# flanglet/kanzi-cpp

Hardware: AMD Instinct MI355X
Metric: encode+decode MB/s on the synthetic stand-in for silesia.tar (bit-exact) (higher is better)
Workload: dtype u8

## Files before the change

kanzi-cpp_amd/csrc/bwt_fwd.hip:

```cpp
#include "common.hpp"
#include "stages.hpp"
#include "bwt_common.hpp"

#include <cstdlib>
#include <cstring>
#include <algorithm>
#include <cmath>
#include "prims.hpp"
#include <chrono>
#include <vector>

namespace knz {

constexpr u32 SM_TS = 1792;
constexpr u32 SM_WIN = 2048;
constexpr u32 SM_G = 256;
constexpr u32 MED_CAP = 8192;
constexpr u32 MED_LO_CAP = 2048;
constexpr u32 SUPER_CAP = 8192;
constexpr int GATHER_THREADS = 512;
constexpr u32 GATHER_ROWS = 16;
static_assert(MED_CAP <= GATHER_ROWS * GATHER_THREADS, "k_bwt_f_gather_desc judges a medium group from one batch of loads");
constexpr u32 LARGE_OS_MIN = 1000000;
constexpr u32 NO_BIT = 0x7FFFFFFFu;
// ... 904 lines not shown
        else for (u32 i0 = 0; i0 < d.y; i0 += GATHER_ROWS * GATHER_THREADS)
            unsplit = gather_rows<(int)GATHER_ROWS>(v, d.x + i0, d.y - i0, off, bb, be, judge, key0, &sDiff);
        if (threadIdx.x == 0) {
            descInfo[g] = make_uint2(bb, lab);
            if (unsplit) {
                v.medStage[d.x >> 8] = d; desc[g] = make_uint2(d.x, 0u);
                if (v.verdictNow) v.verdictNow[d.x >> 8] = make_uint2(key0, verdict_word(v.round, (off == h && key0 != 0u) ? VERDICT_PLAIN : VERDICT_WHOLE, d.y));
            }
            if (stats) {
                atomicAdd(&v.counters[CNT_STAT_MED], d.y); atomicAdd(&v.counters[CNT_STAT_MED_GROUPS], 1u);
                if (unsplit) { atomicAdd(&v.counters[CNT_STAT_UNSPLIT], 1u); atomicAdd(&v.counters[CNT_STAT_UNSPLIT_MEMBERS], d.y); }
            }
        }
        __syncthreads();
    }
}

__device__ __forceinline__ bool sleep_target(const FwdView& v, const uint2* __restrict__ desc, u32 nDesc, u32 lab, u32 bb, bool plain, u32& start, u32& key)
{
    u32 lo = 0, hi = nDesc;
    while (lo < hi) { const u32 mid = (lo + hi) >> 1; if (desc[mid].x <= lab) lo = mid + 1; else hi = mid; }
    if (lo == 0) return false;
    start = desc[lo - 1].x;
    const uint2 t = v.verdictWas[start >> 8];
    const u32 status = (t.y >> 16) & 3u;
    if ((t.y >> 24) != v.round - 1u || (plain ? status != VERDICT_PLAIN : status == 0u) || lab - start >= (t.y & 0xFFFFu)) return false;
    key = t.x;
    return lab_old(v, v.SA[start], bb) == lab;
}

__global__ __launch_bounds__(256) void k_bwt_f_med_sleep(FwdView v, uint2* __restrict__ desc, u32 nDesc, int stats)
{
    const u32 g = blockIdx.x * 256 + threadIdx.x;
    if (g >= nDesc) return;
    const uint2 d = desc[g];
    if (d.y <= SM_G || d.y > MED_CAP) return;
    const uint2 was = v.verdictWas[d.x >> 8];
    if (was.y != verdict_word(v.round - 1u, VERDICT_PLAIN, d.y)) return;
    if (v.rtbits && ((v.rtbits[d.x >> 5] >> (d.x & 31)) & 1u)) return;
    const u32 bb = v.base[find_block(v.base, v.nBlocks, d.x)];
    u32 s1, k1, s2, k2;
    if (!sleep_target(v, desc, nDesc, bb + was.x - 1u, bb, true, s1, k1) || s1 == d.x) return;
    if (!sleep_target(v, desc, nDesc, bb + k1 - 1u, bb, false, s2, k2) || s2 == d.x) return;
    v.verdictNow[d.x >> 8] = make_uint2(k1, verdict_word(v.round, VERDICT_PLAIN, d.y));
    v.medStage[d.x >> 8] = d;
    desc[g] = make_uint2(d.x, 0u);
    if (stats) {
        atomicAdd(&v.counters[CNT_STAT_MED], d.y); atomicAdd(&v.counters[CNT_STAT_MED_GROUPS], 1u);
        atomicAdd(&v.counters[CNT_STAT_UNSPLIT], 1u); atomicAdd(&v.counters[CNT_STAT_UNSPLIT_MEMBERS], d.y);
        atomicAdd(&v.counters[CNT_STAT_ASLEEP], 1u); atomicAdd(&v.counters[CNT_STAT_ASLEEP_MEMBERS], d.y);
    }
}

template <int THREADS, int ROWS>
struct MedLds {
    static constexpr int WAVES = THREADS / 64;
    static constexpr u32 CAP = (u32)ROWS * THREADS;
    u32 oK[CAP];
    u32 oV[CAP];
    u32 cnt[WAVES * 256];
    u32 fb[CAP / 32];
    int pm[CAP / 32];
    u32 pn[CAP / 32];
    u32 wtot[WAVES];
    u32 wtot2[WAVES];
    u32 oldLab;
    u32 blkBase;
};

template <int THREADS, int ROWS>
__device__ __forceinline__ u32 med_block_sum(MedLds<THREADS, ROWS>& L, u32 x)
{
    const u32 s = wave_sum(x);
    if ((threadIdx.x & 63) == 0) L.wtot[threadIdx.x >> 6] = s;
    __syncthreads();
    u32 tot = 0;
    for (int w = 0; w < THREADS / 64; w++) tot += L.wtot[w];
    __syncthreads();
    return tot;
}

template <int THREADS, int ROWS>
__device__ __forceinline__ void med_radix_sort(MedLds<THREADS, ROWS>& L, u32 n, int npass)
{
    constexpr int WAVES = THREADS / 64;
    const int tid = (int)threadIdx.x, lane = tid & 63, wave = tid >> 6;
    const unsigned long long ltMask = (lane == 0) ? 0ull : (~0ull >> (64 - lane));
    u32* cntw = L.cnt + wave * 256;
    const int R = (int)((n + THREADS - 1) / THREADS);
    const u32 waveBase = (u32)wave * (u32)R * 64u;
    for (int pass = 0; pass < npass; pass++) {
        const int shift = 8 * pass;
        for (int q = lane; q < 256; q += 64) cntw[q] = 0;
        u32 key[ROWS], val[ROWS], pre[ROWS];
#pragma unroll
        for (int r = 0; r < ROWS; r++) {
            key[r] = 0xFFFFFFFFu; val[r] = 0; pre[r] = 0;
            if (r < R) {
                const u32 idx = waveBase + (u32)r * 64u + (u32)lane;
                if (idx < n) { key[r] = L.oK[idx]; val[r] = L.oV[idx]; }
                const u32 dg = (key[r] >> shift) & 255u;
                const unsigned long long peers = prims::digit_peers_fast(true, dg);
                const u32 pop = (u32)__popcll(peers);
                const u32 rnk = (u32)__popcll(peers & ltMask);
                const int leader = __ffsll((long long)peers) - 1;
                u32 old = 0;
                if (lane == leader) { old = cntw[dg]; cntw[dg] = old + pop; }
                old = (u32)__shfl((int)old, leader, 64);
                pre[r] = old + rnk;
            }
        }
        __syncthreads();
        {
            constexpr int TPD = THREADS / 256;
            const int dg = tid / TPD, w0 = (tid % TPD) * 4;
            const u32 c0 = L.cnt[(w0 + 0) * 256 + dg], c1 = L.cnt[(w0 + 1) * 256 + dg], c2 = L.cnt[(w0 + 2) * 256 + dg], c3 = L.cnt[(w0 + 3) * 256 + dg];
            const u32 sum = c0 + c1 + c2 + c3;
            const u32 incl = wave_incl_scan(sum);
            if (lane == 63) L.wtot[wave] = incl;
            __syncthreads();
            u32 wbase = 0;
            for (int w = 0; w < wave; w++) wbase += L.wtot[w];
            const u32 excl = wbase + incl - sum;
            L.cnt[(w0 + 0) * 256 + dg] = excl;
            L.cnt[(w0 + 1) * 256 + dg] = excl + c0;
            L.cnt[(w0 + 2) * 256 + dg] = excl + c0 + c1;
            L.cnt[(w0 + 3) * 256 + dg] = excl + c0 + c1 + c2;
        }
        __syncthreads();
#pragma unroll
        for (int r = 0; r < ROWS; r++) {
            if (r < R) {
                const u32 dg = (key[r] >> shift) & 255u;
                const u32 pos = cntw[dg] + pre[r];
                if (pos < n) {
                    L.oK[pos] = key[r];
                    L.oV[pos] = val[r];
                }
            }
        }
        __syncthreads();
    }
    (void)WAVES;
}

template <int THREADS, int ROWS>
__device__ __forceinline__ void med_write_back(MedLds<THREADS, ROWS>& L, const FwdView& v, u32 gs, u32 n, uint2* __restrict__ medNext, uint2* __restrict__ largeNext)
{
    constexpr u32 CAP = (u32)ROWS * THREADS;
    const int tid = (int)threadIdx.x, lane = tid & 63;
    const int nWords = (int)((n + 31) >> 5);
    if (tid < (int)(CAP / 32)) {
        u32 bits = 0;
        if (tid < nWords) {
            const u32 i0 = (u32)tid * 32u;
            u32 prev = (i0 == 0) ? 0u : L.oK[i0 - 1];
            for (u32 k = 0; k < 32; k++) {
                const u32 i = i0 + k;
                if (i >= n) break;
                const u32 cur = L.oK[i];
                if (i == 0 || cur != prev) bits |= 1u << k;
                prev = cur;
            }
        }
        L.fb[tid] = bits;
        L.pm[tid] = bits ? (tid * 32 + 31 - __clz((int)bits)) : -1;
        L.pn[tid] = bits ? (u32)(tid * 32 + __ffs((int)bits) - 1) : n;
    }
    __syncthreads();
    if (tid < 64) {
        constexpr int WPL = (int)(CAP / 32) / 64;
        int run = -1;
        for (int k = 0; k < WPL; k++) { const int x = L.pm[tid * WPL + k]; run = x > run ? x : run; }
        int incl = run;
        for (int o = 1; o < 64; o <<= 1) { const int t = __shfl_up(incl, (unsigned)o, 64); if (tid >= o) incl = t > incl ? t : incl; }
        int carry = __shfl_up(incl, 1u, 64);
        if (tid == 0) carry = -1;
        for (int k = 0; k < WPL; k++) { const int x = L.pm[tid * WPL + k]; carry = x > carry ? x : carry; L.pm[tid * WPL + k] = carry; }
        u32 runn = n;
        for (int k = WPL - 1; k >= 0; k--) { const u32 x = L.pn[tid * WPL + k]; runn = x < runn ? x : runn; }
        u32 incn = runn;
        for (int o = 1; o < 64; o <<= 1) { const u32 t = (u32)__shfl_down((int)incn, (unsigned)o, 64); if (tid + o < 64) incn = t < incn ? t : incn; }
        u32 carn = (u32)__shfl_down((int)incn, 1u, 64);
        if (tid == 63) carn = n;
        for (int k = WPL - 1; k >= 0; k--) { const u32 x = L.pn[tid * WPL + k]; carn = x < carn ? x : carn; L.pn[tid * WPL + k] = carn; }
    }
    __syncthreads();
    u32 surv = 0;
    const u32 oldLab = L.oldLab;
    __shared__ ClassAgg A;
    agg_init(A);
    __syncthreads();
    int hKind[ROWS];
    u32 hLocal[ROWS], hSize[ROWS];
#pragma unroll
    for (int r = 0; r < ROWS; r++) hKind[r] = -1;
    int row = 0;
    for (u32 i = (u32)tid; i < n; i += THREADS, row++) {
        const u32 w = i >> 5, bit = i & 31;
        const u32 lowmask = (bit == 31) ? 0xFFFFFFFFu : ((2u << bit) - 1u);
        const u32 word = L.fb[w];
        const u32 mm = word & lowmask;
        const u32 hd = mm ? (w * 32 + 31 - (u32)__clz((int)mm)) : (u32)L.pm[w - 1];
// ... 19 lines not shown
        if (hKind[r] >= 0) agg_write(A, v, hKind[r], hLocal[r], gs + (u32)tid + (u32)r * THREADS, hSize[r], largeNext, (uint2*)nullptr);
    if (tid < nWords && L.fb[tid]) {
        const u32 off = gs + (u32)tid * 32u;
        const u32 sh = off & 31;
        atomicOr(&v.gnew[off >> 5], L.fb[tid] << sh);
        if (sh && (L.fb[tid] >> (32 - sh))) atomicOr(&v.gnew[(off >> 5) + 1], L.fb[tid] >> (32 - sh));
    }
}

template <int THREADS, int ROWS>
__device__ __forceinline__ void med_majority_write_back(MedLds<THREADS, ROWS>& L, const FwdView& v, u32 gs, u32 n, u32 nOth, u32 c, u32 less, u32 m)
{
    const int tid = (int)threadIdx.x;
    const u32 oldLab = L.oldLab;
    (void)n; (void)m;
    const u32 mStart = gs + less;
    const u32 rel = oldLab - gs;
    const u32 mLab = (c <= SM_G) ? mStart : ((rel >= less && rel < less + c) ? oldLab : mStart + (c >> 1));
    for (u32 i = (u32)tid; i < c; i += THREADS) {
        const u32 gp = L.oV[nOth + i];
        v.SA[mStart + i] = gp;
        if (mLab != oldLab) lab_set(v, gp, L.blkBase, mLab, oldLab);
    }
    u32 surv = 0;
    if (tid == 0) {
        if (less != 0) atomicOr(&v.gnew[mStart >> 5], 1u << (mStart & 31));
        if (c > SM_G) v.medStage[mStart >> 8] = make_uint2(mStart, c);
        else if (c > 1) surv = 1;
    }
    if ((u32)tid < nOth) {
        const u32 t = (u32)tid;
        const u32 key = L.oK[t];
        u32 hd = t, e = t + 1;
        while (hd > 0 && L.oK[hd - 1] == key) hd--;
        while (e < nOth && L.oK[e] == key) e++;
        const u32 size = e - hd;
        const u32 shift = (t < less) ? 0u : c;
        const u32 slot = gs + t + shift, hdSlot = gs + hd + shift;
        const u32 relO = rel - shift;
        const u32 lab = (size <= SM_G) ? hdSlot : ((oldLab >= hdSlot && oldLab < hdSlot + size) ? oldLab : hdSlot + (size >> 1));
        (void)relO;
        const u32 gp = L.oV[t];
        v.SA[slot] = gp;
        if (lab != oldLab) lab_set(v, gp, L.blkBase, lab, oldLab);
        if (t == hd) {
            if (hdSlot != gs) atomicOr(&v.gnew[hdSlot >> 5], 1u << (hdSlot & 31));
            if (size > SM_G) v.medStage[hdSlot >> 8] = make_uint2(hdSlot, size);
            else if (size > 1) surv = 1;
        }
    }
    if (__ballot(surv != 0) != 0 && (tid & 63) == 0) v.counters[CNT_SMALL_LEFT] = 1;
}

template <int THREADS, int ROWS, bool STATS>
__device__ __forceinline__ void med_sort_group(MedLds<THREADS, ROWS>& L, const FwdView& v, u32 gs, u32 n, uint2 info, int npass, bool storeKeys,
                                               uint2* __restrict__ medNext, uint2* __restrict__ largeNext, uint4* __restrict__ superList)
{
    constexpr int WAVES = THREADS / 64;
    const int tid = (int)threadIdx.x, lane = tid & 63, wave = tid >> 6;
    const unsigned long long ltMask = (lane == 0) ? 0ull : (~0ull >> (64 - lane));
    if (tid == 0) { L.oldLab = info.y; L.blkBase = info.x; }
    const u32 ka = L.oK[n >> 2], kb = L.oK[n >> 1], kc = L.oK[(n >> 2) * 3];
    const u32 m = (ka == kc) ? ka : kb;
    u32 c = 0;
    for (u32 i = (u32)tid; i < n; i += THREADS) c += (L.oK[i] == m) ? 1u : 0u;
    c = med_block_sum(L, c);
    if (c < n && 2 * c >= n && n <= SUPER_CAP && m == info.y - info.x + 1u) {
        if (tid == 0) { const u32 at = atomicAdd(&v.counters[CNT_SUPER], 1u); superList[at] = make_uint4(gs, n, info.x, info.y); }
        if (storeKeys) for (u32 i = (u32)tid; i < n; i += THREADS) v.K[gs + i] = L.oK[i];
        __syncthreads();
        return;
    }
    if (STATS && tid == 0 && c == n) { atomicAdd(&v.counters[CNT_STAT_UNSPLIT], 1u); atomicAdd(&v.counters[CNT_STAT_UNSPLIT_MEMBERS], n); }
    if (c < n) {
        if (2 * c >= n) {
            const int R = (int)((n + THREADS - 1) / THREADS);
            const u32 waveBase = (u32)wave * (u32)R * 64u;
            u32 key[ROWS], val[ROWS], pos[ROWS];
            u32 runO = 0, runE = 0;
#pragma unroll
            for (int r = 0; r < ROWS; r++) {
                key[r] = m; val[r] = 0; pos[r] = 0xFFFFFFFFu;
                if (r < R) {
                    const u32 idx = waveBase + (u32)r * 64u + (u32)lane;
                    const bool valid = idx < n;
                    if (valid) { key[r] = L.oK[idx]; val[r] = L.oV[idx]; }
                    const bool oth = valid && key[r] != m, same = valid && key[r] == m;
                    const unsigned long long bo = __ballot(oth), be = __ballot(same);
                    if (oth) pos[r] = runO + (u32)__popcll(bo & ltMask);
                    if (same) pos[r] = 0x80000000u | (runE + (u32)__popcll(be & ltMask));
                    runO += (u32)__popcll(bo);
                    runE += (u32)__popcll(be);
                }
            }
            if (lane == 0) { L.wtot[wave] = runO; L.wtot2[wave] = runE; }
            __syncthreads();
            u32 baseO = 0, baseE = 0, nOth = 0;
            for (int w = 0; w < WAVES; w++) { if (w < wave) { baseO += L.wtot[w]; baseE += L.wtot2[w]; } nOth += L.wtot[w]; }
#pragma unroll
            for (int r = 0; r < ROWS; r++) {
                if (r < R && pos[r] != 0xFFFFFFFFu) {
                    const u32 at = (pos[r] & 0x80000000u) ? (nOth + baseE + (pos[r] & 0x7FFFFFFFu)) : (baseO + pos[r]);
                    L.oK[at] = key[r];
                    L.oV[at] = val[r];
                }
            }
            __syncthreads();
            if (nOth <= (u32)THREADS) {
                u32 kk = 0, vv = 0, at = 0;
                if ((u32)tid < nOth) {
                    kk = L.oK[tid]; vv = L.oV[tid];
                    for (u32 j = 0; j < nOth; j++) { const u32 kj = L.oK[j]; at += (kj < kk || (kj == kk && j < (u32)tid)) ? 1u : 0u; }
                }
                __syncthreads();
                if ((u32)tid < nOth) { L.oK[at] = kk; L.oV[at] = vv; }
                __syncthreads();
                u32 lessQ = 0;
                if ((u32)tid < nOth) lessQ = (L.oK[tid] < m) ? 1u : 0u;
                lessQ = med_block_sum(L, lessQ);
                if (tid == 0) { L.oldLab = info.y; L.blkBase = info.x; if (STATS) { atomicAdd(&v.counters[CNT_STAT_MAJ], 1u); atomicAdd(&v.counters[CNT_STAT_MAJ_MEMBERS], n); } }
                __syncthreads();
                med_majority_write_back<THREADS, ROWS>(L, v, gs, n, nOth, c, lessQ, m);
                __syncthreads();
                return;
            } else {
                med_radix_sort<THREADS, ROWS>(L, nOth, npass);
            }
            u32 less = 0;
            for (u32 i = (u32)tid; i < nOth; i += THREADS) less += (L.oK[i] < m) ? 1u : 0u;
            less = med_block_sum(L, less);
#pragma unroll
            for (int k = 0; k < ROWS; k++) {
                const u32 i = (u32)tid + (u32)k * THREADS;
                if (i < n) { key[k] = L.oK[i]; val[k] = L.oV[i]; }
            }
            __syncthreads();
#pragma unroll
            for (int k = 0; k < ROWS; k++) {
                const u32 i = (u32)tid + (u32)k * THREADS;
                if (i < n) {
                    const u32 at = (i < less) ? i : (i < nOth ? i + c : less + (i - nOth));
                    L.oK[at] = key[k];
                    L.oV[at] = val[k];
                }
            }
            __syncthreads();
        } else {
            med_radix_sort<THREADS, ROWS>(L, n, npass);
        }
    }
    med_write_back<THREADS, ROWS>(L, v, gs, n, medNext, largeNext);
    __syncthreads();
}

template <int THREADS, int ROWS, bool STATS>
__global__ __launch_bounds__(THREADS, (THREADS >= 1024 ? 4 : THREADS / 128)) void k_bwt_f_sort_medium(FwdView v, const uint2* __restrict__ desc, u32 nDesc, int npass, u32 minLen,
                                                               uint2* __restrict__ medNext, uint2* __restrict__ largeNext, const uint2* __restrict__ descInfo,
                                                               uint4* __restrict__ superList)
{
    constexpr u32 CAP = (u32)ROWS * THREADS;
    __shared__ MedLds<THREADS, ROWS> L;
    const int tid = (int)threadIdx.x;

    for (u32 g = blockIdx.x; g < nDesc; g += gridDim.x) {
        const uint2 d = desc[g];
        const u32 gs = d.x, n = d.y;
        if (n <= minLen || n > CAP) continue;
        const uint2 info = descInfo[g];
        {
            u32 k[ROWS], p[ROWS];
#pragma unroll
            for (int r = 0; r < ROWS; r++) { const u32 i = (u32)tid + (u32)r * THREADS; k[r] = 0; p[r] = 0; if (i < n) { k[r] = v.K[gs + i]; p[r] = v.SA[gs + i]; } }
#pragma unroll
            for (int r = 0; r < ROWS; r++) { const u32 i = (u32)tid + (u32)r * THREADS; if (i < n) { L.oK[i] = k[r]; L.oV[i] = p[r]; } }
        }
        __syncthreads();
        med_sort_group<THREADS, ROWS, STATS>(L, v, gs, n, info, npass, false, medNext, largeNext, superList);
    }
}

template <int THREADS, int ROWS, bool STATS>
__global__ __launch_bounds__(THREADS, 4) void k_bwt_f_medium_fused(FwdView v, const uint2* __restrict__ desc, const u32* __restrict__ classIdx, u32 nClass, u32 h, int npass,
                                                               int skip, uint2* __restrict__ medNext, uint2* __restrict__ largeNext, uint4* __restrict__ superList)
{
    constexpr u32 CAP = (u32)ROWS * THREADS;
    __shared__ MedLds<THREADS, ROWS> L;
    __shared__ u32 sDiff;
    const int tid = (int)threadIdx.x;
    const u32 xcd = blockIdx.x & 7, lanesPerXcd = gridDim.x >> 3, slot = blockIdx.x >> 3;
    const u32 per = (nClass + 7) / 8;
    const u32 lo = xcd * per, hi = (lo + per < nClass) ? lo + per : nClass;
    if (tid == 0) sDiff = 0;
    __syncthreads();
    for (u32 g = lo + slot; g < hi; g += lanesPerXcd) {
        const uint2 d = desc[classIdx[g]];
        const u32 gs = d.x, n = d.y;
        if (n <= SM_G || n > CAP) continue;
        const int blk = find_block(v.base, v.nBlocks, gs);
        const u32 bb = v.base[blk], be = v.base[blk + 1];
        u32 off = h;
        if (v.rtbits && ((v.rtbits[gs >> 5] >> (gs & 31)) & 1u)) { const u32 r = v.ovr[gs]; off = r > h ? r : h; }
        const u32 gp0 = v.SA[gs];
        const u32 lab = lab_old(v, gp0, bb), key0 = gather_key(v, gp0, off, bb, be);
        const bool judge = skip && lab - gs < n;
        u32 gp[ROWS], key[ROWS];
#pragma unroll
        for (int r = 0; r < ROWS; r++) { const u32 i = (u32)tid + (u32)r * THREADS; gp[r] = (i < n) ? v.SA[gs + i] : bb; }
#pragma unroll
        for (int r = 0; r < ROWS; r++) { const u32 i = (u32)tid + (u32)r * THREADS; key[r] = (i < n) ? gather_key(v, gp[r], off, bb, be) : key0; }
        bool unsplit = false;
        if (judge) {
            bool diff = false;
#pragma unroll
            for (int r = 0; r < ROWS; r++) diff = diff || key[r] != key0;
            if (__ballot(diff) != 0 && (tid & 63) == 0) sDiff = 1;
            __syncthreads();
            unsplit = sDiff == 0;
        }
        if (tid == 0) {
            if (unsplit) {
                v.medStage[gs >> 8] = d;
                if (v.verdictNow) v.verdictNow[gs >> 8] = make_uint2(key0, verdict_word(v.round, (off == h && key0 != 0u) ? VERDICT_PLAIN : VERDICT_WHOLE, n));
            }
            if (STATS) {
                atomicAdd(&v.counters[CNT_STAT_MED], n); atomicAdd(&v.counters[CNT_STAT_MED_GROUPS], 1u);
                if (unsplit) { atomicAdd(&v.counters[CNT_STAT_UNSPLIT], 1u); atomicAdd(&v.counters[CNT_STAT_UNSPLIT_MEMBERS], n); }
            }
        }
        if (unsplit) { __syncthreads(); continue; }
#pragma unroll
        for (int r = 0; r < ROWS; r++) { const u32 i = (u32)tid + (u32)r * THREADS; if (i < n) { L.oK[i] = key[r]; L.oV[i] = gp[r]; } }
        __syncthreads();
        if (tid == 0) sDiff = 0;
        med_sort_group<THREADS, ROWS, STATS>(L, v, gs, n, make_uint2(bb, lab), npass, true, medNext, largeNext, superList);
    }
}

__global__ __launch_bounds__(1024) void k_bwt_f_super(FwdView v, const uint4* __restrict__ superList, u32 h, int npass, uint2* __restrict__ medNext, uint2* __restrict__ largeNext)
{
    constexpr int THREADS = 1024, ROWS = 8;
    constexpr u32 CAP = (u32)ROWS * THREADS;
    __shared__ MedLds<THREADS, ROWS> L;
    __shared__ u16 nxt[CAP];
    __shared__ u16 cn[CAP];
    __shared__ u16 trEnd[CAP];
    __shared__ u32 sEnds;
    __shared__ u32 sMoved[2];
    __shared__ u32 sCmax;
    const int tid = (int)threadIdx.x, lane = tid & 63;
    const unsigned long long ltMask = (lane == 0) ? 0ull : (~0ull >> (64 - lane));
    const u32 nList = v.counters[CNT_SUPER];
    for (u32 g = blockIdx.x; g < nList; g += gridDim.x) {
        const uint4 d = superList[g];
        const u32 gs = d.x, n = d.y;
        {
            u32 k[ROWS], p[ROWS];
#pragma unroll
            for (int r = 0; r < ROWS; r++) { const u32 i = (u32)tid + (u32)r * THREADS; k[r] = 0; p[r] = 0; if (i < n) { k[r] = v.K[gs + i]; p[r] = v.SA[gs + i]; } }
#pragma unroll
            for (int r = 0; r < ROWS; r++) { const u32 i = (u32)tid + (u32)r * THREADS; if (i < n) { L.oK[i] = k[r]; L.oV[i] = p[r]; } }
        }
        if (tid == 0) { sEnds = 0; sCmax = 0; L.oldLab = d.w; L.blkBase = d.z; }
        __syncthreads();
        const u32 m = d.w - d.z + 1u;
        u32 link = h;
        if (v.rtbits && ((v.rtbits[gs >> 5] >> (gs & 31)) & 1u)) { const u32 r = v.ovr[gs]; link = r > h ? r : h; }
#pragma unroll 4
        for (int r = 0; r < ROWS; r++) {
            const u32 i = (u32)tid + (u32)r * THREADS;
            if (i >= n) continue;
            u32 to = i, one = 0;
            if (L.oK[i] == m) {
                const u32 target = L.oV[i] + link;
                u32 lo = i + 1, hi = n;
                while (lo < hi) { const u32 mid = (lo + hi) >> 1; if (L.oV[mid] < target) lo = mid + 1; else hi = mid; }
                if (lo < n && L.oV[lo] == target) { to = lo; one = 1; }
            }
            nxt[i] = (u16)to; cn[i] = (u16)one;
        }
        __syncthreads();
        for (u32 span = 1, it = 0; span < n; span <<= 1, it ^= 1) {
            u32 a[ROWS], b[ROWS];
            bool moved = false;
#pragma unroll
            for (int r = 0; r < ROWS; r++) {
                const u32 i = (u32)tid + (u32)r * THREADS;
                a[r] = 0; b[r] = 0;
// ... 810 lines not shown
        u32 word = 0, have = 0;
#pragma unroll
        for (u32 k = 0; k < 4; k++) {
            const u32 q = 4 * w + k;
            if (q >= qLo && q < qHi) {
                const u32 rr = q - qLo;
                const u32 r = rr + (rr >= r0 ? 1u : 0u);
                const u32 p = SA[bb + r] - bb;
                word |= (u32)s[p - 1] << (8 * k);
                have |= 1u << k;
            }
        }
        if (have == 0xF && al) reinterpret_cast<u32*>(d)[w] = word;
        else for (u32 k = 0; k < 4; k++) if ((have >> k) & 1) d[4 * w + k] = (u8)(word >> (8 * k));
    }
    if (blockIdx.x == 0 && threadIdx.x == 0) {
        d[hdr] = s[n - 1];
        const u32 st = n / (u32)chunks;
        const u32 step = ((u32)chunks * st == n) ? st : st + 1;
        const u32 logNbChunks = (u32)ilog2_u32((u32)chunks);
        d[0] = (u8)((logNbChunks << 2) | (pIndexSize - 1));
        u32 idx = 1;
        for (int k = 0; k < chunks; k++) {
            const u32 prim = lab_cur(fv, bb + (u32)k * step, bb) - bb;
            for (int sh = (int)(pIndexSize - 1) * 8; sh >= 0; sh -= 8) d[idx++] = (u8)(prim >> sh);
        }
        newLen[b] = hdr + n;
    }
}

__global__ __launch_bounds__(256) void k_bwt_f_med_flags(const uint2* __restrict__ stage, u32 nSlots, u32* __restrict__ flags)
{
    const u32 i = blockIdx.x * 256 + threadIdx.x;
    if (i >= nSlots) return;
    const u32 n = stage[i].y;
    flags[i] = (n != 0 && n <= MED_LO_CAP) ? 1u : 0u;
    flags[nSlots + i] = (n > MED_LO_CAP) ? 1u : 0u;
}

__global__ __launch_bounds__(256) void k_bwt_f_med_compact(uint2* __restrict__ stage, u32 nSlots, const u32* __restrict__ prefix, uint2* __restrict__ medNext,
                                                           u32 at, u32* __restrict__ idxLo, u32 atLo, u32* __restrict__ idxHi, u32 atHi, u32* __restrict__ nLoOut)
{
    const u32 i = blockIdx.x * 256 + threadIdx.x;
    if (i >= nSlots) return;
    const u32 nLo = prefix[nSlots];
    if (i == 0) *nLoOut = nLo;
    const uint2 d = stage[i];
    if (d.y == 0) return;
    const u32 pLo = prefix[i], pHi = prefix[nSlots + i] - nLo, g = at + pLo + pHi;
    medNext[g] = d; stage[i] = make_uint2(0u, 0u);
    if (d.y <= MED_LO_CAP) idxLo[atLo + pLo] = g; else idxHi[atHi + pHi] = g;
}

struct FwdTuning { int nsym; int noRunRound; int runFallback; int stats; int link; int plainLabels; int noPack; int noUnsplitSkip; int noGroupSleep; int noMediumFuse; int runSort; };
static FwdTuning& fwd_tuning()
{
    static FwdTuning t = [] {
        FwdTuning x; x.nsym = 0; x.noRunRound = 0; x.runFallback = 0; x.stats = 0; x.link = 1; x.plainLabels = 0; x.noPack = 0; x.noUnsplitSkip = 0; x.noGroupSleep = 0; x.noMediumFuse = 0; x.runSort = 0;
        if (getenv("KNZ_BWT_PLAIN_LABELS")) x.plainLabels = 1;
        if (getenv("KNZ_BWT_NO_PACK")) x.noPack = 1;
        if (getenv("KNZ_BWT_NO_UNSPLIT_SKIP")) x.noUnsplitSkip = 1;
        if (getenv("KNZ_BWT_NO_GROUP_SLEEP")) x.noGroupSleep = 1;
        if (getenv("KNZ_BWT_NO_MEDIUM_FUSE")) x.noMediumFuse = 1;
        if (const char* e = getenv("KNZ_BWT_RUN_SORT")) x.runSort = atoi(e);
        if (const char* e = getenv("KNZ_BWT_LINK")) x.link = atoi(e);
        if (getenv("KNZ_BWT_STATS")) x.stats = 1;
        if (const char* e = getenv("KNZ_BWT_NSYM")) x.nsym = atoi(e);
        if (getenv("KNZ_BWT_NO_RUN_ROUND")) x.noRunRound = 1;
        if (getenv("KNZ_BWT_RUN_FALLBACK")) x.runFallback = 1;
        return x;
    }();
    return t;
}
int bwt_forward_tune(const char* key, int value)
{
    FwdTuning& t = fwd_tuning();
    if (!strcmp(key, "rs_onesweep")) { prims::rs_onesweep_knob().store(value); return 0; }
    if (!strcmp(key, "bwt_nsym")) t.nsym = value;
    else if (!strcmp(key, "bwt_no_run_round")) t.noRunRound = value;
    else if (!strcmp(key, "bwt_run_fallback")) t.runFallback = value;
    else if (!strcmp(key, "bwt_stats")) t.stats = value;
    else if (!strcmp(key, "bwt_link")) t.link = value;
    else if (!strcmp(key, "bwt_plain_labels")) t.plainLabels = value;
    else if (!strcmp(key, "bwt_no_pack")) t.noPack = value;
    else if (!strcmp(key, "bwt_no_unsplit_skip")) t.noUnsplitSkip = value;
    else if (!strcmp(key, "bwt_no_group_sleep")) t.noGroupSleep = value;
    else if (!strcmp(key, "bwt_no_medium_fuse")) t.noMediumFuse = value;
    else if (!strcmp(key, "bwt_run_sort")) t.runSort = value;
    else return -1;
    return 0;
}

struct FwdScratch {
    u64* keysA; u64* keysB;
    u32* valsA; u32* valsB;
    u32* SA; u32* ISA; u32* K; u64* ISA2;
    u32* t0; u32* t1; u32* t2; u32* t3;
    u32* gbits; u32* gnew; u32* rtbits; u32* ovr; size_t gbitsWords;
    uint2* med[2]; uint2* medStage; uint2* medVerdict[2]; u32* medFlags; u32* medPrefix; u32* medIdxLo; u32* medIdxHi; size_t medSlots; uint2* descInfo; uint2* large[2]; uint2* runList; uint4* superList; u32* ebits;
    u32* loff; u32* lbase;
    u32* survTile;
    u32* linkedTile;
    u32* base;
    u32* counters;
    u32* seg2;
    void* scanTmp;
    void* rsMem;
    u32* byteHist;
    u32* classTab; u32* rbits; u32* rcount; u32* rprefix;
    u32* runPos; u32* runE; u32* runL; u32* sE; u32* rcnt; u32* moff;
    u64* runKeysA; u64* runKeysB; u64* sKey;
    u32* runTileStart; u32* runColTab;
    size_t maxRuns;
};

static size_t fwd_align(size_t x) { return (x + 255) & ~(size_t)255; }

static size_t fwd_carve(u8* p, int nBlocks, size_t total, FwdScratch* w, u32 VS)
{
    u8* q = p;
    auto take = [&](size_t sz) { u8* r = q; q += fwd_align(sz); return r; };
    const size_t maxMed = 2 * (total / (SM_G + 1) + 2), maxLarge = total / (MED_CAP + 1) + 2;
    w->gbitsWords = ((total + 64) / 64 + SM_WIN / 64 + 4) * 2 + 128;
    w->keysA = (u64*)take(8 * total); w->keysB = (u64*)take(8 * total);
    w->valsA = (u32*)take(4 * total); w->valsB = (u32*)take(4 * total);
    w->SA = (u32*)take(4 * total); w->ISA = (u32*)take(4 * total); w->K = (u32*)take(4 * total);
    w->ISA2 = (VS <= (1u << LAB_BITS)) ? (u64*)take(8 * total) : (u64*)nullptr;
    w->t0 = (u32*)take(4 * total); w->t1 = (u32*)take(4 * total); w->t2 = (u32*)take(4 * total); w->t3 = (u32*)take(4 * total);
    w->gbits = (u32*)take(4 * w->gbitsWords);
    w->gnew = (u32*)take(4 * w->gbitsWords);
    w->rtbits = (u32*)take(4 * w->gbitsWords);
    w->ovr = (u32*)take(4 * total);
    w->med[0] = (uint2*)take(8 * maxMed); w->med[1] = (uint2*)take(8 * maxMed);
    w->medSlots = total / 256 + 2;
    w->medStage = (uint2*)take(8 * w->medSlots); w->medFlags = (u32*)take(8 * w->medSlots + 64); w->medPrefix = (u32*)take(8 * w->medSlots + 64);
    w->medIdxLo = (u32*)take(4 * maxMed); w->medIdxHi = (u32*)take(4 * maxMed);
    w->medVerdict[0] = (uint2*)take(16 * w->medSlots); w->medVerdict[1] = w->medVerdict[0] + w->medSlots;
    w->large[0] = (uint2*)take(8 * maxLarge); w->large[1] = (uint2*)take(8 * maxLarge);
    w->runList = (uint2*)take(8 * maxMed);
    w->superList = (uint4*)take(16 * maxMed);
    w->descInfo = (uint2*)take(8 * maxMed);
// ... 231 lines not shown
        compact_medium(w.med[cur]);
        { KScope ks_("k_bwt_f_probe"); hipLaunchKernelGGL(k_bwt_f_probe_scan, dim3(256), dim3(256), 0, s, v, w.med[cur], (u32)nsym, v.rtbits, probeCand); }
        if (fetch(0, CNT_ROUND_SLOTS)) return -1;
        surv = hp[CNT_SMALL_LEFT]; nMed = hp[CNT_MED]; nMedLo = hp[CNT_MED_LO]; nLarge = hp[CNT_LARGE]; largeElems = hp[CNT_LARGE_MEMBERS];
        if (const u32 nCand = hp[CNT_PROBE_CAND]) {
            enable_run_tiebits();
            hipMemsetAsync(w.counters, 0, 4 * CNT_PROBE_SLOTS, s);
            { KScope ks_("k_bwt_f_probe");
              hipLaunchKernelGGL(k_bwt_f_probe, dim3(std::min<u32>(nCand, 4096)), dim3(512), 0, s, bv, v, w.med[cur], probeCand, nCand, (u32)nsym, w.med[cur ^ 1], w.large[cur], w.ovr, w.rtbits);
              merge_bits(); }
            compact_medium(w.med[cur], nMed, nMedLo);
            if (fetch(0, CNT_MED_LO + 1)) return -1;
            surv |= hp[CNT_SMALL_LEFT]; nMed += hp[CNT_MED]; nMedLo += hp[CNT_MED_LO];
        }
        if (tune.stats) fprintf(stderr, "after round 0 (nsym %d, total %u): run groups %u (%u members); small left %u, medium %u, large %u (%u members); run members placed directly %u, sorted %u\n",
                                nsym, total, nRun, runElems, surv, nMed, nLarge, largeElems, (nRun && runDirect) ? runElems : 0u, (nRun && !runDirect) ? runElems : 0u);
        statT = std::chrono::steady_clock::now();
        return 0;
    }
    void link_step()
    {
        KScope ks_("k_bwt_f_link");
        u32* posflag = w.ebits; u32* linked = w.rbits; u32* rev = w.rcount; u32* sufRev = w.rprefix;
        const bool trial = link.mode == LinkPlan::TRIAL; linkTr.n = 0;
        if (trial) { linkTr.blk[linkTr.n++] = 0; if (st.nBlocks >= 5) linkTr.blk[linkTr.n++] = st.nBlocks / 2; if (st.nBlocks >= 3) linkTr.blk[linkTr.n++] = st.nBlocks - 1; }
        const u32 nW = total / 32 + 1;
        hipMemsetAsync(posflag, 0, 4 * (size_t)nW, s);
        hipMemsetAsync(linked, 0, 4 * ((size_t)nTiles * (SM_TS / 32) + 64), s);
        enable_run_tiebits();
        const u32 nTrial = (u32)std::min<u64>((u64)nTiles, ((u64)bv.VS + SM_TS - 1) / SM_TS + 2);
        const dim3 gridL(trial ? nTrial : nTiles, (unsigned)(linkTr.n ? linkTr.n : 1));
        hipLaunchKernelGGL(k_bwt_f_link_small, gridL, dim3(256), 0, s, v, posflag, linked, tune.stats, 1u, w.linkedTile, linkTr);
        hipLaunchKernelGGL(k_bwt_f_link_zeros, GRID1(nW), posflag, nW, rev);
        prims::launch_scan<prims::SCAN_MIN_INCL>(s, rev, sufRev, nW, nullptr, w.scanTmp);
        hipLaunchKernelGGL(k_bwt_f_link_apply, gridL, dim3(256), 0, s, v, posflag, sufRev, nW, linked, h, w.ovr, w.rtbits, 1u, linkTr);
    }
    void sort_small(bool linked)
    {
        KScope ks_("k_bwt_f_sort_small");
        u32* survTile = tune.link ? w.survTile : nullptr;
        if (v.ISA2 && pbits <= 23 && !tune.noPack) hipLaunchKernelGGL(k_bwt_f_small_fused<true>, dim3(nTiles), dim3(256), 0, s, v, h, survTile, tune.stats);
        else if (v.ISA2) hipLaunchKernelGGL(k_bwt_f_small_fused<false>, dim3(nTiles), dim3(256), 0, s, v, h, survTile, tune.stats);
        else hipLaunchKernelGGL(k_bwt_f_sort_small, dim3(nTiles), dim3(256), 0, s, v, survTile);
        if (linked) hipLaunchKernelGGL(k_bwt_f_link_payoff, dim3(1), dim3(256), 0, s, v, w.linkedTile, w.survTile, nTiles, 1u, w.counters + CNT_LINKED, linkTr);
        if (tune.link) prims::launch_scan<prims::SCAN_SUM_EXCL>(s, w.survTile, w.survTile, nTiles, nullptr, w.scanTmp, w.counters + CNT_TIED);
    }
    void sort_medium()
    {
        const int npass = (kbits + 7) / 8, nxt = cur ^ 1;
        if (medFuse) {
            KScope ks_("k_bwt_f_medium_fused"); const int skip = tune.noUnsplitSkip ? 0 : 1; const u32 nMedHi = nMed - nMedLo;
            const auto fuse256 = tune.stats ? k_bwt_f_medium_fused<256, 8, true> : k_bwt_f_medium_fused<256, 8, false>;
            const auto fuse512 = tune.stats ? k_bwt_f_medium_fused<512, 16, true> : k_bwt_f_medium_fused<512, 16, false>;
            if (nMedLo) hipLaunchKernelGGL(fuse256, dim3(std::min<u32>((nMedLo + 7) / 8 * 8, 2048)), dim3(256), 0, s, v, w.med[cur], w.medIdxLo, nMedLo, h, npass, skip, w.med[nxt], w.large[nxt], w.superList);
            if (nMedHi) hipLaunchKernelGGL(fuse512, dim3(std::min<u32>((nMedHi + 7) / 8 * 8, 1024)), dim3(512), 0, s, v, w.med[cur], w.medIdxHi, nMedHi, h, npass, skip, w.med[nxt], w.large[nxt], w.superList);
        } else { KScope ks_("k_bwt_f_sort_medium"); const dim3 gridM(std::min<u32>(nMed, 8192));
          const auto sort256 = tune.stats ? k_bwt_f_sort_medium<256, 8, true> : k_bwt_f_sort_medium<256, 8, false>;
          const auto sort512 = tune.stats ? k_bwt_f_sort_medium<512, 16, true> : k_bwt_f_sort_medium<512, 16, false>;
          hipLaunchKernelGGL(sort256, gridM, dim3(256), 0, s, v, w.med[cur], nMed, npass, SM_G, w.med[nxt], w.large[nxt], w.descInfo, w.superList);
          hipLaunchKernelGGL(sort512, gridM, dim3(512), 0, s, v, w.med[cur], nMed, npass, MED_LO_CAP, w.med[nxt], w.large[nxt], w.descInfo, w.superList); }
        { KScope ks_("k_bwt_f_super"); hipLaunchKernelGGL(k_bwt_f_super, dim3(std::min<u32>(nMed, 512)), dim3(1024), 0, s, v, w.superList, h, npass, w.med[nxt], w.large[nxt]); }
    }
    template <class KEY> void large_keys()
    {
        { KScope ks_("k_bwt_f_large_prefix"); hipLaunchKernelGGL(k_bwt_f_large_prefix, dim3(1), dim3(1024), 0, s, w.large[cur], nLarge, w.loff, w.base, st.nBlocks, w.lbase); }
        KScope ks_("k_bwt_f_large_keys");
        hipLaunchKernelGGL(k_bwt_f_large_keys<KEY>, GRID1(largeElems), v, w.large[cur], nLarge, w.loff, largeElems, h, kbits, reinterpret_cast<KEY*>(keysFree), w.valsA);
    }
    template <class KEY> void sort_large(int lbits)
    {
        KEY* ka = reinterpret_cast<KEY*>(keysFree); KEY* kb = reinterpret_cast<KEY*>(keysFree2); int r;
        { KScope ks_("k_bwt_f_sort_large");
          r = sort_one_segment<KEY, true>(largeElems, ka, kb, w.valsA, w.valsB, 0, kbits + lbits, largeElems >= LARGE_OS_MIN); }
        const KEY* sk = r ? kb : ka; const u32* sv = r ? w.valsB : w.valsA;
        { KScope ks_("k_bwt_f_large_flags"); hipLaunchKernelGGL(k_bwt_f_large_flags<KEY>, GRID1(largeElems), sk, largeElems, w.t0, w.t2); }
        bounds(largeElems, true);
        { KScope ks_("k_bwt_f_large_place");
          hipLaunchKernelGGL(k_bwt_f_large_place<KEY>, GRID1(largeElems), v, w.large[cur], w.loff, largeElems, kbits, sk, sv, w.t1, w.t3, w.med[cur ^ 1], w.large[cur ^ 1], w.lbase); }
    }
    int end_round()
    {
        { KScope ks_("k_bwt_f_merge_bits"); merge_bits(); }
        compact_medium(w.med[cur ^ 1]);
        if (fetch(0, CNT_ROUND_SLOTS)) return -1;
        surv = hp[CNT_SMALL_LEFT]; nMed = hp[CNT_MED]; nMedLo = hp[CNT_MED_LO]; nLarge = hp[CNT_LARGE]; largeElems = hp[CNT_LARGE_MEMBERS]; survMembers = hp[CNT_TIED];
        if (tune.stats) {
            std::vector<u32> hs(nTiles); u32 activeTiles = 0;
            if (tune.link && hipMemcpyAsync(hs.data(), w.survTile, 4 * (size_t)nTiles, hipMemcpyDeviceToHost, s) == hipSuccess && hipStreamSynchronize(s) == hipSuccess) {
                for (u32 t = 0; t + 1 < nTiles; t++) activeTiles += hs[t + 1] != hs[t] ? 1u : 0u;
                fprintf(stderr, "  windows with tied small groups after the round: %u of %u\n", activeTiles, nTiles);
            }
            const std::chrono::steady_clock::time_point now = std::chrono::steady_clock::now();
            fprintf(stderr, "round h=%u (%.3f ms): small members worked on %u in %u groups, medium members %u; after it: small left %u, medium groups %u, large %u (%u members); %u groups took the chain round; %u small members still tied\n",
                    h, std::chrono::duration<double, std::milli>(now - statT).count(), hp[CNT_STAT_SMALL], hp[CNT_STAT_SMALL_GROUPS], hp[CNT_STAT_MED], surv, nMed, nLarge, largeElems,
                    hp[CNT_SUPER], hp[CNT_TIED]);
            fprintf(stderr, "  medium groups worked on %u (%u members): all keys equal in %u (%u members)%s, majority path %u (%u members), asleep %u (%u members)\n", hp[CNT_STAT_MED_GROUPS], hp[CNT_STAT_MED],
                    hp[CNT_STAT_UNSPLIT], hp[CNT_STAT_UNSPLIT_MEMBERS], tune.noUnsplitSkip ? "" : " -- left alone", hp[CNT_STAT_MAJ], hp[CNT_STAT_MAJ_MEMBERS], hp[CNT_STAT_ASLEEP], hp[CNT_STAT_ASLEEP_MEMBERS]);
            statT = now;
        }
        cur ^= 1; h <<= 1;
        return 0;
    }
    int round()
    {
        if (h > bv.VS) return -5;
        { KScope ks_("k_bwt_f_round"); hipMemsetAsync(w.counters, 0, 4 * CNT_ROUND_SLOTS, s); }
        if (++v.round > 255) return -5;
        const bool linked = surv && tune.link && h >= (u32)(tune.link > 1 ? tune.link : 32)
                            && link.next(h, survMembers, total, hp[CNT_LINKED], hp[CNT_LINK_TIED], tune.stats);
        if (linked) link_step();
        if (surv && !v.ISA2) { KScope ks_("k_bwt_f_gather_small"); hipLaunchKernelGGL(k_bwt_f_gather_small, dim3(nTiles), dim3(256), 0, s, v, h, tune.stats); }
        if (groupSleep) { v.verdictNow = w.medVerdict[v.round & 1]; v.verdictWas = w.medVerdict[(v.round & 1) ^ 1]; }
        if (groupSleep && nMed && v.round >= 2) { KScope ks_("k_bwt_f_med_sleep"); hipLaunchKernelGGL(k_bwt_f_med_sleep, GRID1(nMed), v, w.med[cur], nMed, tune.stats); }
        if (nMed && !medFuse) { KScope ks_("k_bwt_f_gather_desc"); hipLaunchKernelGGL(k_bwt_f_gather_desc, dim3(1024), dim3(GATHER_THREADS), 0, s, v, w.med[cur], nMed, h, w.descInfo, tune.stats, tune.noUnsplitSkip ? 0 : 1); }
// ... 33 lines not shown
```

Baseline: 6968.

## Resolve periodic medium groups in-block via pointer-jumping chain ranking

Adds med_chain_round, which handles 'super' medium groups (majority key equal to the group's own label, i.e. periodic runs) inside the fused medium kernel. It links members by position offset, ranks the chains by pointer jumping, sorts the chain ends by tail key and re-sorts the members with a composite key, instead of deferring them to the separate k_bwt_f_super kernel. The super kernel launch is now skipped when the fused path is active and the chain path is enabled by default. This adds binary searches, several LDS passes and extra radix sorts per periodic group, and relies on the ranking being bit-exact. A small asm barrier on threadIdx in write-back is also added.

```diff
diff --git a/kanzi-cpp_amd/csrc/bwt_fwd.hip b/kanzi-cpp_amd/csrc/bwt_fwd.hip
--- a/kanzi-cpp_amd/csrc/bwt_fwd.hip
+++ b/kanzi-cpp_amd/csrc/bwt_fwd.hip
@@ -980,6 +980,15 @@
     }
 }
 
+__device__ __forceinline__ int local_tid()
+{
+    int t = (int)threadIdx.x;
+#if defined(__HIP_DEVICE_COMPILE__) && !defined(KNZ_EMU)
+    asm volatile("" : "+v"(t));
+#endif
+    return t;
+}
+
 template <int THREADS, int ROWS>
 struct MedLds {
     static constexpr int WAVES = THREADS / 64;
@@ -1076,7 +1085,7 @@
 __device__ __forceinline__ void med_write_back(MedLds<THREADS, ROWS>& L, const FwdView& v, u32 gs, u32 n, uint2* __restrict__ medNext, uint2* __restrict__ largeNext)
 {
     constexpr u32 CAP = (u32)ROWS * THREADS;
-    const int tid = (int)threadIdx.x, lane = tid & 63;
+    const int tid = local_tid(), lane = tid & 63;
     const int nWords = (int)((n + 31) >> 5);
     if (tid < (int)(CAP / 32)) {
         u32 bits = 0;
@@ -1202,8 +1211,138 @@
     if (__ballot(surv != 0) != 0 && (tid & 63) == 0) v.counters[CNT_SMALL_LEFT] = 1;
 }
 
+template <int THREADS, int ROWS>
+__device__ __forceinline__ bool med_chain_round(MedLds<THREADS, ROWS>& L, const FwdView& v, u32 gs, u32 n, u32 m, u32 link, int npass)
+{
+    constexpr u32 CAP = (u32)ROWS * THREADS, HALF = CAP / 2;
+    static_assert(CAP <= 0x2000u, "index and chain length of a member: 13 bits each");
+    __shared__ u32 sEnds, sAt, sCmax, sMoved[2];
+    const int tid = (int)threadIdx.x, lane = tid & 63;
+    const unsigned long long ltMask = (lane == 0) ? 0ull : (~0ull >> (64 - lane));
+    if (tid == 0) { sEnds = 0; sAt = 0; sCmax = 0; }
+    __syncthreads();
+    u32 w[ROWS];
+    {
+        u32 nE = 0;
+#pragma unroll
+        for (int r = 0; r < ROWS; r++) {
+            const u32 i = (u32)tid + (u32)r * THREADS;
+            w[r] = i;
+            if (i < n) {
+                bool found = false;
+                if (L.oK[i] == m) {
+                    const u32 target = L.oV[i] + link;
+                    u32 lo = i + 1, hi = n;
+                    if (lo < n && L.oV[lo] == target) hi = lo;
+                    while (lo < hi) { const u32 mid = (lo + hi) >> 1; if (L.oV[mid] < target) lo = mid + 1; else hi = mid; }
+                    if (lo < n && L.oV[lo] == target) { w[r] = lo | (1u << 16); found = true; }
+                }
+                nE += found ? 0u : 1u;
+            }
+        }
+        nE = wave_sum(nE);
+        if (lane == 0 && nE) atomicAdd(&sEnds, nE);
+    }
+    __syncthreads();
+    const u32 nEnds = sEnds;
+    if (nEnds > HALF) return false;
+#pragma unroll
+    for (int r = 0; r < ROWS; r++) { const u32 i = (u32)tid + (u32)r * THREADS; if (i < n) L.oV[i] = w[r]; }
+    __syncthreads();
+    for (u32 span = 1, it = 0; span < n; span <<= 1, it ^= 1) {
+        bool moved = false;
+#pragma unroll
+        for (int r = 0; r < ROWS; r++) {
+            const u32 i = (u32)tid + (u32)r * THREADS;
+            if (i < n) {
+                const u32 wi = L.oV[i], j = wi & 0xFFFFu, wj = L.oV[j], k = wj & 0xFFFFu, wk = L.oV[k];
+                w[r] = (wk & 0xFFFFu) | (((wi >> 16) + (wj >> 16) + (wk >> 16)) << 16);
+                moved = moved || ((wk & 0xFFFFu) != k);
+            }
+        }
+        if (tid == 0) sMoved[it] = 0;
+        __syncthreads();
+        if (moved) sMoved[it] = 1;
+#pragma unroll
+        for (int r = 0; r < ROWS; r++) { const u32 i = (u32)tid + (u32)r * THREADS; if (i < n) L.oV[i] = w[r]; }
+        __syncthreads();
+        if (!sMoved[it]) break;
+    }
+    {
+        u32 cm = 0;
+#pragma unroll
+        for (int r = 0; r < ROWS; r++) {
+            const u32 i = (u32)tid + (u32)r * THREADS;
+            const bool in = i < n;
+            const u32 cc = w[r] >> 16;
+            const u32 tail = in ? L.oK[w[r] & 0xFFFFu] : m;
+            if (in && tail < m) w[r] |= 0x80000000u;
+            cm = (in && cc > cm) ? cc : cm;
+            const bool isEnd = in && cc == 0;
+            const unsigned long long bal = __ballot(isEnd);
+            u32 base0 = 0;
+            if (lane == 0 && bal) base0 = atomicAdd(&sAt, (u32)__popcll(bal));
+            base0 = (u32)__shfl((int)base0, 0, 64);
+            if (isEnd) { const u32 at = base0 + (u32)__popcll(bal & ltMask); L.oV[at] = i; L.oV[HALF + at] = tail; }
+        }
+        cm = wave_max(cm);
+        if (lane == 0 && cm) atomicMax(&sCmax, cm);
+    }
+    __syncthreads();
+    for (u32 j = (u32)tid; j < nEnds; j += THREADS) L.oK[j] = L.oV[HALF + j];
+    __syncthreads();
+#pragma unroll
+    for (int r = 0; r < ROWS; r++) { const u32 i = (u32)tid + (u32)r * THREADS; if (r < ROWS / 2) L.oK[HALF + i] = w[r]; else L.oV[i] = w[r]; }
+    if (nEnds <= (u32)THREADS) {
+        u32 kk = 0, vv = 0, at = 0;
+        if ((u32)tid < nEnds) {
+            kk = L.oK[tid]; vv = L.oV[tid];
+            for (u32 j = 0; j < nEnds; j++) { const u32 kj = L.oK[j]; at += (kj < kk || (kj == kk && j < (u32)tid)) ? 1u : 0u; }
+        }
+        __syncthreads();
+        if ((u32)tid < nEnds) { L.oK[at] = kk; L.oV[at] = vv; }
+        __syncthreads();
+    } else {
+        med_radix_sort<THREADS, ROWS>(L, nEnds, npass);
+    }
+#pragma unroll
+    for (int r = 0; r < ROWS; r++) { const u32 i = (u32)tid + (u32)r * THREADS; w[r] = (r < ROWS / 2) ? L.oK[HALF + i] : L.oV[i]; }
+    __syncthreads();
+    for (u32 j = (u32)tid; j < nEnds; j += THREADS) {
+        const u32 key = L.oK[j];
+        u32 lo = 0, hi = j;
+        while (lo < hi) { const u32 mid = (lo + hi) >> 1; if (L.oK[mid] < key) lo = mid + 1; else hi = mid; }
+        const u32 e = L.oV[j];
+        if (e < HALF) L.oK[HALF + e] = lo; else L.oV[e] = lo;
+    }
+    __syncthreads();
+    const u32 cmax = sCmax;
+    const u32 trBits = bitlen_u32(nEnds ? nEnds - 1 : 0), hiBits = bitlen_u32(2u * cmax + 1u);
+#pragma unroll
+    for (int r = 0; r < ROWS; r++) {
+        const u32 i = (u32)tid + (u32)r * THREADS;
+        if (i < n) {
+            const u32 e = w[r] & 0xFFFFu, cc = (w[r] >> 16) & 0x7FFFu;
+            const u32 hiKey = (w[r] >> 31) ? cc : (2u * cmax + 1u - cc);
+            w[r] = (hiKey << trBits) | (e < HALF ? L.oK[HALF + e] : L.oV[e]);
+        }
+    }
+    __syncthreads();
+#pragma unroll
+    for (int r = 0; r < ROWS; r++) { const u32 i = (u32)tid + (u32)r * THREADS; if (i < n) { L.oK[i] = w[r]; L.oV[i] = i; } }
+    __syncthreads();
+    med_radix_sort<THREADS, ROWS>(L, n, (int)((hiBits + trBits + 7) / 8));
+#pragma unroll
+    for (int r = 0; r < ROWS; r++) { const u32 i = (u32)tid + (u32)r * THREADS; if (i < n) w[r] = v.SA[gs + L.oV[i]]; }
+    __syncthreads();
+#pragma unroll
+    for (int r = 0; r < ROWS; r++) { const u32 i = (u32)tid + (u32)r * THREADS; if (i < n) L.oV[i] = w[r]; }
+    __syncthreads();
+    return true;
+}
+
 template <int THREADS, int ROWS, bool STATS>
-__device__ __forceinline__ void med_sort_group(MedLds<THREADS, ROWS>& L, const FwdView& v, u32 gs, u32 n, uint2 info, int npass, bool storeKeys,
+__device__ __forceinline__ void med_sort_group(MedLds<THREADS, ROWS>& L, const FwdView& v, u32 gs, u32 n, uint2 info, int npass, bool storeKeys, u32 chainLink,
                                                uint2* __restrict__ medNext, uint2* __restrict__ largeNext, uint4* __restrict__ superList)
 {
     constexpr int WAVES = THREADS / 64;
@@ -1215,14 +1354,19 @@
     u32 c = 0;
     for (u32 i = (u32)tid; i < n; i += THREADS) c += (L.oK[i] == m) ? 1u : 0u;
     c = med_block_sum(L, c);
+    bool chained = false;
     if (c < n && 2 * c >= n && n <= SUPER_CAP && m == info.y - info.x + 1u) {
-        if (tid == 0) { const u32 at = atomicAdd(&v.counters[CNT_SUPER], 1u); superList[at] = make_uint4(gs, n, info.x, info.y); }
-        if (storeKeys) for (u32 i = (u32)tid; i < n; i += THREADS) v.K[gs + i] = L.oK[i];
-        __syncthreads();
-        return;
+        if (chainLink == 0u) {
+            if (tid == 0) { const u32 at = atomicAdd(&v.counters[CNT_SUPER], 1u); superList[at] = make_uint4(gs, n, info.x, info.y); }
+            if (storeKeys) for (u32 i = (u32)tid; i < n; i += THREADS) v.K[gs + i] = L.oK[i];
+            __syncthreads();
+            return;
+        }
+        chained = med_chain_round<THREADS, ROWS>(L, v, gs, n, m, chainLink, npass);
+        if (chained && tid == 0) atomicAdd(&v.counters[CNT_SUPER], 1u);
     }
     if (STATS && tid == 0 && c == n) { atomicAdd(&v.counters[CNT_STAT_UNSPLIT], 1u); atomicAdd(&v.counters[CNT_STAT_UNSPLIT_MEMBERS], n); }
-    if (c < n) {
+    if (c < n && !chained) {
         if (2 * c >= n) {
             const int R = (int)((n + THREADS - 1) / THREADS);
             const u32 waveBase = (u32)wave * (u32)R * 64u;
@@ -1325,13 +1469,13 @@
             for (int r = 0; r < ROWS; r++) { const u32 i = (u32)tid + (u32)r * THREADS; if (i < n) { L.oK[i] = k[r]; L.oV[i] = p[r]; } }
         }
         __syncthreads();
-        med_sort_group<THREADS, ROWS, STATS>(L, v, gs, n, info, npass, false, medNext, largeNext, superList);
+        med_sort_group<THREADS, ROWS, STATS>(L, v, gs, n, info, npass, false, 0u, medNext, largeNext, superList);
     }
 }
 
 template <int THREADS, int ROWS, bool STATS>
 __global__ __launch_bounds__(THREADS, 4) void k_bwt_f_medium_fused(FwdView v, const uint2* __restrict__ desc, const u32* __restrict__ classIdx, u32 nClass, u32 h, int npass,
-                                                               int skip, uint2* __restrict__ medNext, uint2* __restrict__ largeNext, uint4* __restrict__ superList)
+                                                               int skip, int chainList, uint2* __restrict__ medNext, uint2* __restrict__ largeNext, uint4* __restrict__ superList)
 {
     constexpr u32 CAP = (u32)ROWS * THREADS;
     __shared__ MedLds<THREADS, ROWS> L;
@@ -1382,7 +1526,7 @@
         for (int r = 0; r < ROWS; r++) { const u32 i = (u32)tid + (u32)r * THREADS; if (i < n) { L.oK[i] = key[r]; L.oV[i] = gp[r]; } }
         __syncthreads();
         if (tid == 0) sDiff = 0;
-        med_sort_group<THREADS, ROWS, STATS>(L, v, gs, n, make_uint2(bb, lab), npass, true, medNext, largeNext, superList);
+        med_sort_group<THREADS, ROWS, STATS>(L, v, gs, n, make_uint2(bb, lab), npass, true, chainList ? 0u : off, medNext, largeNext, superList);
     }
 }
 
@@ -2299,17 +2443,18 @@
     if (d.y <= MED_LO_CAP) idxLo[atLo + pLo] = g; else idxHi[atHi + pHi] = g;
 }
 
-struct FwdTuning { int nsym; int noRunRound; int runFallback; int stats; int link; int plainLabels; int noPack; int noUnsplitSkip; int noGroupSleep; int noMediumFuse; int runSort; };
+struct FwdTuning { int nsym; int noRunRound; int runFallback; int stats; int link; int plainLabels; int noPack; int noUnsplitSkip; int noGroupSleep; int noMediumFuse; int runSort; int chainList; };
 static FwdTuning& fwd_tuning()
 {
     static FwdTuning t = [] {
-        FwdTuning x; x.nsym = 0; x.noRunRound = 0; x.runFallback = 0; x.stats = 0; x.link = 1; x.plainLabels = 0; x.noPack = 0; x.noUnsplitSkip = 0; x.noGroupSleep = 0; x.noMediumFuse = 0; x.runSort = 0;
+        FwdTuning x; x.nsym = 0; x.noRunRound = 0; x.runFallback = 0; x.stats = 0; x.link = 1; x.plainLabels = 0; x.noPack = 0; x.noUnsplitSkip = 0; x.noGroupSleep = 0; x.noMediumFuse = 0; x.runSort = 0; x.chainList = 0;
         if (getenv("KNZ_BWT_PLAIN_LABELS")) x.plainLabels = 1;
         if (getenv("KNZ_BWT_NO_PACK")) x.noPack = 1;
         if (getenv("KNZ_BWT_NO_UNSPLIT_SKIP")) x.noUnsplitSkip = 1;
         if (getenv("KNZ_BWT_NO_GROUP_SLEEP")) x.noGroupSleep = 1;
         if (getenv("KNZ_BWT_NO_MEDIUM_FUSE")) x.noMediumFuse = 1;
         if (const char* e = getenv("KNZ_BWT_RUN_SORT")) x.runSort = atoi(e);
+        if (const char* e = getenv("KNZ_BWT_CHAIN_LIST")) x.chainList = atoi(e);
         if (const char* e = getenv("KNZ_BWT_LINK")) x.link = atoi(e);
         if (getenv("KNZ_BWT_STATS")) x.stats = 1;
         if (const char* e = getenv("KNZ_BWT_NSYM")) x.nsym = atoi(e);
@@ -2334,6 +2479,7 @@
     else if (!strcmp(key, "bwt_no_group_sleep")) t.noGroupSleep = value;
     else if (!strcmp(key, "bwt_no_medium_fuse")) t.noMediumFuse = value;
     else if (!strcmp(key, "bwt_run_sort")) t.runSort = value;
+    else if (!strcmp(key, "bwt_chain_list")) t.chainList = value;
     else return -1;
     return 0;
 }
@@ -2671,14 +2817,14 @@
             KScope ks_("k_bwt_f_medium_fused"); const int skip = tune.noUnsplitSkip ? 0 : 1; const u32 nMedHi = nMed - nMedLo;
             const auto fuse256 = tune.stats ? k_bwt_f_medium_fused<256, 8, true> : k_bwt_f_medium_fused<256, 8, false>;
             const auto fuse512 = tune.stats ? k_bwt_f_medium_fused<512, 16, true> : k_bwt_f_medium_fused<512, 16, false>;
-            if (nMedLo) hipLaunchKernelGGL(fuse256, dim3(std::min<u32>((nMedLo + 7) / 8 * 8, 2048)), dim3(256), 0, s, v, w.med[cur], w.medIdxLo, nMedLo, h, npass, skip, w.med[nxt], w.large[nxt], w.superList);
-            if (nMedHi) hipLaunchKernelGGL(fuse512, dim3(std::min<u32>((nMedHi + 7) / 8 * 8, 1024)), dim3(512), 0, s, v, w.med[cur], w.medIdxHi, nMedHi, h, npass, skip, w.med[nxt], w.large[nxt], w.superList);
+            if (nMedLo) hipLaunchKernelGGL(fuse256, dim3(std::min<u32>((nMedLo + 7) / 8 * 8, 2048)), dim3(256), 0, s, v, w.med[cur], w.medIdxLo, nMedLo, h, npass, skip, tune.chainList ? 1 : 0, w.med[nxt], w.large[nxt], w.superList);
+            if (nMedHi) hipLaunchKernelGGL(fuse512, dim3(std::min<u32>((nMedHi + 7) / 8 * 8, 1024)), dim3(512), 0, s, v, w.med[cur], w.medIdxHi, nMedHi, h, npass, skip, tune.chainList ? 1 : 0, w.med[nxt], w.large[nxt], w.superList);
         } else { KScope ks_("k_bwt_f_sort_medium"); const dim3 gridM(std::min<u32>(nMed, 8192));
           const auto sort256 = tune.stats ? k_bwt_f_sort_medium<256, 8, true> : k_bwt_f_sort_medium<256, 8, false>;
           const auto sort512 = tune.stats ? k_bwt_f_sort_medium<512, 16, true> : k_bwt_f_sort_medium<512, 16, false>;
           hipLaunchKernelGGL(sort256, gridM, dim3(256), 0, s, v, w.med[cur], nMed, npass, SM_G, w.med[nxt], w.large[nxt], w.descInfo, w.superList);
           hipLaunchKernelGGL(sort512, gridM, dim3(512), 0, s, v, w.med[cur], nMed, npass, MED_LO_CAP, w.med[nxt], w.large[nxt], w.descInfo, w.superList); }
-        { KScope ks_("k_bwt_f_super"); hipLaunchKernelGGL(k_bwt_f_super, dim3(std::min<u32>(nMed, 512)), dim3(1024), 0, s, v, w.superList, h, npass, w.med[nxt], w.large[nxt]); }
+        if (!medFuse || tune.chainList) { KScope ks_("k_bwt_f_super"); hipLaunchKernelGGL(k_bwt_f_super, dim3(std::min<u32>(nMed, 512)), dim3(1024), 0, s, v, w.superList, h, npass, w.med[nxt], w.large[nxt]); }
     }
     template <class KEY> void large_keys()
     {
```

After: 7185 (median of 6 runs). 3.1% higher.
